# aosokin/os2d

Measured on AMD Instinct MI355X. Metric: query-image-pairs/s (1280-px input, ResNet50, N-class), higher is better.
Workload: dtype fftx3 (as fft; the per-bin complex GEMM on the fp16 MFMA with spectra split into fp16 hi+lo, 3 MFMAs per product, fp32 accumulate)

## Files before the change

include/os2d_hip.h:

```cpp
#ifndef OS2D_HIP_H
#define OS2D_HIP_H

#include <stddef.h>

#ifdef __cplusplus
extern "C" {
#endif

#define OS2D_ABI_VERSION 9

#define OS2D_PRECISION_F32 0
#define OS2D_PRECISION_F16X3 1
#define OS2D_PRECISION_F16X2 2

#define OS2D_PRECISION_FFT 3

#define OS2D_PRECISION_FFT32 5

#define OS2D_PRECISION_FFTX3 4

int os2d_abi_version(void);

const char* os2d_last_error(void);

// ... 20 lines not shown
int os2d_pack_conv_f16x3(int layer , int P, const float* w, const float* b, const float* bn_weight,
                         const float* bn_bias, const float* bn_running_mean, const float* bn_running_var, float bn_eps,
                         const int* weight_exp, const int* in_exp, const int* out_exp, void* packed_w, float* packed_b,
                         void* stream);

size_t os2d_class_split_bytes(int B, int C);
int os2d_class_split(const float* qp, void* qs, int B, int C, void* stream);

#define OS2D_STATUS_F16_RANGE 1
int os2d_head_forward_ex(const float* fm, const float* qp, const void* w1, const float* b1, const void* w2,
                         const float* b2, const void* w3, const float* b3, int A, int B, int C, int H, int W, int P,
                         int inverse, int stride, int rec_field, float* loc, float* cls, float* corners,
                         void* workspace, size_t workspace_bytes, void* stream, int precision, const void* qs,
                         void** stage_events, int* chunk_classes, int* status, const float* wspec, const float* twQ,
                         const float* twP);
void os2d_debug_set_dump(void* stream, int slot, void* dst, size_t bytes);
int os2d_prof_event_create(void** ev);
int os2d_prof_event_destroy(void* ev);
int os2d_prof_event_elapsed_ms(void* begin, void* end, float* ms);

int os2d_fm_sumsq(const float* fm, float* sumsq, int A, int C, int H, int W, void* stream);
size_t os2d_plane_floats(int H, int W);
int os2d_corr(const float* fm, const float* qp, const float* sumsq, float* corr, float* rnorm, int A, int B, int C,
              int H, int W, void* stream);
size_t os2d_corr_f16x3_workspace_bytes(int A, int C, int H, int W);
int os2d_corr_f16x3(const float* fm, const void* qs, float* corr, void* rshb, int A, int B, int C, int H, int W,
                    void* workspace, size_t workspace_bytes, void* stream);
size_t os2d_corr_f16x3_packed_workspace_bytes(int A, int B, int C, int H, int W);
int os2d_corr_f16x3_packed(const float* fm, const void* qs, float* corr, float* inv_norm, int A, int B, int C, int H, int W,
                           int form, void* workspace, size_t workspace_bytes, void* stream);
// ... 47 lines not shown
size_t os2d_spectral_weight16_bytes(int C, int nbins);
int os2d_spectral_weights_build(const double* wfold, const double* twP64, const double* twQ64, int C, int Cout, int P, int Q,
                                int nbins, int split, void* out, void* workspace, void* stream);
float os2d_spectral_xscale(int H, int W);
int os2d_spectral_gemm_f16(const void* w16, const float* X, float* Y, int NB, int C, int Cout, int nbins, float xscale,
                           void* stream);

int os2d_dft_sizes(int H, int W, int* P, int* Q, int* nbins, int* tiles);
int os2d_dft_channel_stride(int C);
size_t os2d_dft_matrices_bytes(int P, int Q);
int os2d_dft_matrices_build(const double* twP64, const double* twQ64, int P, int Q, void* out, void* stream);
int os2d_dft_forward(const float* corr, const float* inv_norm, float* X, const void* matrices, int NB, int C, int H, int W,
                     void* stream);
int os2d_dft_inverse(const float* Y, const float* packed_b, void* out, const void* matrices, int NB, int Cout, int H, int W,
                     int* status, void* stream);
int os2d_spectral_weights_build_dft(const double* wfold, const double* twP64, const double* twQ64, int C, int Cout, int P, int Q,
                                    int nbins, void* out, void* workspace, void* stream);
int os2d_spectral_gemm_f16_quads(const void* w16, const float* X, float* Y, int NB, int C, int Cout, int nbins, float xscale,
                                 void* stream);
float os2d_dft_xscale(int H, int W);

#define OS2D_PYRAMID_MAX_LEVELS 16
int os2d_detect_pyramid_supported(int L, int N, int nms_max_batch);
int os2d_detect_pyramid_workspace_bytes(int B, int N, int passes, size_t* bytes);
int os2d_detect_pyramid(const float* const* loc, const float* const* cls, const float* const* corners, int B, int L,
                        const int* hw, int stride, int rec_field, const float* img_wh, const float* scale_xy,
                        float score_threshold, float iou_threshold, int nms_max_batch, int passes, float* out_boxes,
                        float* out_scores, int* out_index, float* out_default, float* out_corners, int* out_count,
                        int* unfinished, void* workspace, size_t workspace_bytes, void* stream);
int os2d_detect_pyramid_merged(const float* const* loc, const float* const* cls, const float* const* corners, int B, int L,
// ... 19 lines not shown
```

os2d_amd/_lib.py:

```python
import ctypes

from . import build
from ._native import NativeLibrary, Os2dLibraryError

ABI_VERSION = 9

_c_float_p = ctypes.c_void_p
_vp = ctypes.c_void_p
_i = ctypes.c_int
_f = ctypes.c_float
_sz = ctypes.c_size_t

SIGNATURES = {
    "os2d_abi_version": (_i, []),
    "os2d_last_error": (ctypes.c_char_p, []),
    "os2d_packed_conv_floats": (_sz, [_i]),
    "os2d_packed_bias_floats": (_sz, [_i]),
    "os2d_pack_conv": (_i, [_i, _i, _vp, _vp, _vp, _vp, _vp, _vp, _f, _vp, _vp, _vp]),
    "os2d_class_prepare": (_i, [_vp, _i, _i, _i, _i, _vp, _vp, _vp]),
    "os2d_head_workspace_bytes": (_i, [_i, _i, _i, _i, _i, _i, ctypes.POINTER(_sz)]),
    "os2d_head_forward": (_i, [_vp] * 8 + [_i] * 9 + [_vp, _vp, _vp, _vp, _sz, _vp]),
    "os2d_packed_conv_bytes": (_sz, [_i, _i]),
    "os2d_pack_conv_f16x3": (_i, [_i, _i, _vp, _vp, _vp, _vp, _vp, _vp, _f, _vp, _vp, _vp, _vp, _vp, _vp]),
    "os2d_rnorm_exp": (_i, []),
# ... 16 lines not shown
    "os2d_fft_inverse": (_i, [_vp, _vp, _vp, _vp, _vp, _i, _i, _i, _i, _vp, _vp]),
    "os2d_fft_inverse_ex": (_i, [_vp, _vp, _vp, _vp, _vp, _i, _i, _i, _i, _vp, _i, _vp]),
    "os2d_dft_sizes": (_i, [_i, _i, ctypes.POINTER(_i), ctypes.POINTER(_i), ctypes.POINTER(_i), ctypes.POINTER(_i)]),
    "os2d_dft_channel_stride": (_i, [_i]),
    "os2d_dft_matrices_bytes": (_sz, [_i, _i]),
    "os2d_dft_matrices_build": (_i, [_vp, _vp, _i, _i, _vp, _vp]),
    "os2d_dft_forward": (_i, [_vp, _vp, _vp, _vp, _i, _i, _i, _i, _vp]),
    "os2d_dft_inverse": (_i, [_vp, _vp, _vp, _vp, _i, _i, _i, _i, _vp, _vp]),
    "os2d_spectral_weights_build_dft": (_i, [_vp, _vp, _vp, _i, _i, _i, _i, _i, _vp, _vp, _vp]),
    "os2d_spectral_gemm_f16_quads": (_i, [_vp, _vp, _vp, _i, _i, _i, _i, _f, _vp]),
    "os2d_dft_xscale": (_f, [_i, _i]),
    "os2d_class_split": (_i, [_vp, _vp, _i, _i, _vp]),
    "os2d_class_split_bytes": (_sz, [_i, _i]),
    "os2d_head_forward_ex": (_i, [_vp] * 8 + [_i] * 9 + [_vp, _vp, _vp, _vp, _sz, _vp, _i, _vp,
                                  ctypes.POINTER(_vp), ctypes.POINTER(_i), _vp, _vp, _vp, _vp]),
    "os2d_head_workspace_bytes_ex": (_i, [_i, _i, _i, _i, _i, _i, _i, ctypes.POINTER(_sz)]),
    "os2d_prof_event_create": (_i, [ctypes.POINTER(_vp)]),
    "os2d_prof_event_destroy": (_i, [_vp]),
    "os2d_prof_event_elapsed_ms": (_i, [_vp, _vp, ctypes.POINTER(_f)]),
    "os2d_fm_sumsq": (_i, [_vp, _vp, _i, _i, _i, _i, _vp]),
    "os2d_plane_floats": (_sz, [_i, _i]),
    "os2d_corr": (_i, [_vp, _vp, _vp, _vp, _vp, _i, _i, _i, _i, _i, _vp]),
    "os2d_corr_normalize": (_i, [_vp, _vp, _i, _i, _i, _vp]),
    "os2d_corr_f16x3_workspace_bytes": (_sz, [_i, _i, _i, _i]),
    "os2d_corr_f16x3": (_i, [_vp, _vp, _vp, _vp, _i, _i, _i, _i, _i, _vp, _sz, _vp]),
    "os2d_corr_f16x3_packed_workspace_bytes": (_sz, [_i, _i, _i, _i, _i]),
    "os2d_corr_f16x3_packed": (_i, [_vp, _vp, _vp, _vp, _i, _i, _i, _i, _i, _i, _vp, _sz, _vp]),
    "os2d_transform_conv": (_i, [_i, _vp, _vp, _vp, _vp, _i, _i, _i, _i, _vp]),
    "os2d_sample_decode": (_i, [_vp, _vp, _i, _i, _i, _i, _i, _i, _i, _vp, _vp, _vp, _vp]),
    "os2d_decode_boxes": (_i, [_vp, _i, _i, _i, _i, _i, _f, _f, _vp, _vp]),
# ... 43 lines not shown
```

os2d_amd/csrc/abi.hip:

```cpp
#include <stdio.h>

#include "../../include/os2d_hip.h"
#include "os2d_common.h"
#include "detect_common.h"
#include <atomic>
#include <mutex>
#include <random>
#include <vector>

namespace {
struct ConvShape {
  int cout, cin, ks, mt;
};
bool conv_shape(int layer, int P, ConvShape* s) {
  switch (layer) {
    case 1: *s = {128, OS2D_K, 7, 128}; return true;
    case 2: *s = {64, 128, 5, 64}; return true;
    case 3: *s = {P, 64, 5, 32}; return true;
    default: return false;
  }
}
size_t align_up(size_t x, size_t a) { return (x + a - 1) / a * a; }

int os2d_conv1_steps_padded() { return 25; }
// ... 366 lines not shown
  if (!boxes || !counts || !keep || !num_keep || !workspace || NC < 1 || N < 1) {
    os2d_set_error("os2d_nms: bad arguments");
    return -1;
  }
  if ((reinterpret_cast<uintptr_t>(boxes) & 15) || (reinterpret_cast<uintptr_t>(workspace) & 15)) {
    os2d_set_error("os2d_nms: boxes and workspace must be 16-byte aligned");
    return -1;
  }
  if (workspace_bytes < (size_t)NC * N * 4 * sizeof(float)) {
    os2d_set_error("os2d_nms: workspace too small");
    return -2;
  }
  return os2d_launch_nms(boxes, counts, NC, N, iou_threshold, keep, num_keep, workspace, os2d_stream(stream));
}

int os2d_head_forward_ex(const float* fm, const float* qp, const void* w1, const float* b1, const void* w2,
                         const float* b2, const void* w3, const float* b3, int A, int B, int C, int H, int W, int P,
                         int inverse, int stride, int rec_field, float* loc, float* cls, float* corners,
                         void* workspace, size_t workspace_bytes, void* stream, int precision, const void* qs,
                         void** stage_events, int* chunk_classes, int* status, const float* wspec, const float* twQ,
                         const float* twP) {
  if (!fm || !qp || !w1 || !b1 || !w2 || !b2 || !w3 || !b3 || !loc || !cls || !corners || !workspace) {
    os2d_set_error("os2d_head_forward: null pointer");
    return -1;
  }
  if (precision != OS2D_PRECISION_F32 && precision != OS2D_PRECISION_F16X3 && precision != OS2D_PRECISION_F16X2 &&
      precision != OS2D_PRECISION_FFT && precision != OS2D_PRECISION_FFTX3 && precision != OS2D_PRECISION_FFT32) {
    os2d_set_error("os2d_head_forward: unknown precision %d", precision);
    return -1;
  }
  int fft_bins = 0, tiles[6] = {1, 1, 0, 0, 0, 0};
  const bool dft = precision == OS2D_PRECISION_FFTX3;
  if (is_freq(precision)) {
    if (!wspec || !twQ || (!dft && !twP)) {
      os2d_set_error("os2d_head_forward: the frequency-domain modes need the weight spectra and the transform tables "
                     "(fft / fft32: twQ, twP; fftx3: the matrices of os2d_dft_matrices_build as twQ)");
      return -1;
    }
    if (!freq_plan(precision, H, W, nullptr, nullptr, &fft_bins, tiles)) {
      os2d_set_error("os2d_head_forward: no transform plan for a %dx%d map", H, W);
      return -3;
    }
  } else if (!direct7_width_ok(W)) {
    return -1;
  }
  const int fft_T = tiles[0] * tiles[1], xch = dft ? OS2D_XSPEC_CPAD : OS2D_K;
  const bool fp32_ops = precision == OS2D_PRECISION_F32 || precision == OS2D_PRECISION_FFT32;
  if (!fp32_ops && !qs) {
    os2d_set_error("os2d_head_forward: precision f16x3 / f16x2 needs the split class operand (os2d_class_split)");
    return -1;
  }
  if (!head_args_ok(A, B, C, H, W, P)) return -1;
  if (stride < 1 || rec_field < 1) {
    os2d_set_error("os2d_head_forward: bad stride/rec_field %d/%d", stride, rec_field);
    return -1;
  }
  if (reinterpret_cast<uintptr_t>(workspace) & 255) {
    os2d_set_error("os2d_head_forward: workspace must be 256-byte aligned");
    return -1;
  }
  const size_t one = carve(A, 1, C, H, W, P, fft_bins, fft_T, xch).total;
// ... 52 lines not shown
    } else {
      if ((rc = os2d_launch_corr(fm, qp + (size_t)b0 * C * OS2D_QROWS, sumsq, corr, fft_bins ? nullptr : rpad, invn, A, bc, C, H, W,
                                 0, st)))
        return rc;
    }
    mark(b0, 1);
    mark(b0, 2);
    if (fft_bins) {
      bool inv_borders = false;
      if (f16) {
        static const bool borders_in_inverse = [] {
          const char* e = getenv("OS2D_BORDERS_IN_INVERSE");
          return !(e && e[0] == '0');
        }();
        inv_borders = dft && borders_in_inverse;
        const int planes = inv_borders ? 0 : NB * 16 * 2;
        if ((planes || sumfx) &&
            (rc = os2d_launch_border_zero_shb_planes_norms(h1, planes, H, W, sumfx, invn, (size_t)NB * H * W, st)))
          return rc;
      } else if ((rc = os2d_launch_border_zero(h1, NB * 128, H, W, st))) {
        return rc;
      }
      mark(b0, 10);
      const int layout = precision == OS2D_PRECISION_FFTX3 ? OS2D_SPECTRA_QUADS : OS2D_SPECTRA_ROWS;
      if (dft) {
        const void* mats = twQ;
        if ((rc = os2d_launch_dft_forward(corr, invn, xspec, mats, NB, OS2D_K, xch, H, W, st))) return rc;
        mark(b0, 11);
        if ((rc = os2d_launch_spectral_gemm_f16(wspec, xspec, yspec, NB * fft_T, OS2D_K, 128, fft_bins,
                                                os2d_spectral_xscale_for(tiles[4], tiles[5]), 1, xch, st)))
          return rc;
        mark(b0, 12);
        if ((rc = os2d_launch_dft_inverse(yspec, b1, 128, h1, mats, NB, 128, H, W, whole_call, inv_borders ? 1 : 0, st))) return rc;
      } else {
        if ((rc = os2d_launch_fft_forward(corr, invn, xspec, twQ, twP, NB, OS2D_K, H, W, st))) return rc;
        mark(b0, 11);
        if ((rc = os2d_launch_spectral_gemm(wspec, xspec, yspec, NB * fft_T, OS2D_K, 128, fft_bins, st))) return rc;
        mark(b0, 12);
        if ((rc = os2d_launch_fft_inverse(yspec, b1, 128, h1, twQ, twP, NB, 128, H, W, whole_call, layout, f16 ? 0 : 1, st))) return rc;
      }
    } else if (f16) {
      if ((rc = os2d_launch_conv_f16x3(1, rpad, w1, b1, whole_call, h1, NB, P, H, W, terms1, st))) return rc;
    } else {
      if ((rc = os2d_launch_conv(1, rpad, static_cast<const float*>(w1), b1, h1, NB, P, H, W, st))) return rc;
    }
    mark(b0, 3);
    mark(b0, 4);
    if (dumps_active() && b0 == 0) {
      const size_t PLb = os2d_plane(H, W);
      dump_slot(stream, 0, corr, (size_t)NB * OS2D_K * H * W * 4);
      if (fft_bins) {
        dump_slot(stream, 1, invn, (size_t)NB * H * W * 4);
        dump_slot(stream, 2, xspec, (size_t)NB * fft_T * OS2D_K * fft_bins * 8);
        dump_slot(stream, 3, yspec, (size_t)NB * fft_T * 128 * fft_bins * 8);
      }
      dump_slot(stream, 4, h1, (size_t)NB * 128 * PLb * 4);
    }
    if (f16) {
      if ((rc = os2d_launch_conv_f16x3(2, h1, w2, b2, whole_call, h2, NB, P, H, W, 3, st))) return rc;
    } else {
      if ((rc = os2d_launch_conv(2, h1, static_cast<const float*>(w2), b2, h2, NB, P, H, W, st))) return rc;
    }
    mark(b0, 5);
    mark(b0, 6);
    if (dumps_active() && b0 == 0) dump_slot(stream, 5, h2, (size_t)NB * 64 * os2d_plane(H, W) * 4);
    static const bool fused_tail_env = [] {
      const char* e = getenv("OS2D_FUSED_TAIL");
      return !(e && e[0] == '0');
    }();
    const bool fused_tail = f16 && fused_tail_env && !dumps_active();
    if (fused_tail) {
      if ((rc = os2d_launch_conv3_sample_decode(h2, w3, b3, corr, NB, H, W, P, inverse, stride, rec_field, bc, B, b0, loc, cls, corners,
                                                flags, epoch, status, st)))
// ... 7 lines not shown
      if ((rc = os2d_launch_conv_f16x3(3, h2, w3, b3, whole_call, params, NB, P, H, W, 3, st))) return rc;
    } else {
      if ((rc = os2d_launch_conv(3, h2, static_cast<const float*>(w3), b3, params, NB, P, H, W, st))) return rc;
    }
    mark(b0, 7);
    mark(b0, 8);
    if (dumps_active() && b0 == 0) dump_slot(stream, 6, params, (size_t)NB * P * H * W * 4);
    if ((rc = os2d_launch_sample_decode(corr, params, NB, H, W, P, inverse, stride, rec_field, bc, B, b0, loc, cls,
                                        corners, fp32_ops ? nullptr : flags, epoch, status, st)))
      return rc;
    mark(b0, 9);
  }
  return 0;
}

int os2d_head_forward(const float* fm, const float* qp, const float* w1, const float* b1, const float* w2,
                      const float* b2, const float* w3, const float* b3, int A, int B, int C, int H, int W, int P,
                      int inverse, int stride, int rec_field, float* loc, float* cls, float* corners, void* workspace,
                      size_t workspace_bytes, void* stream) {
  return os2d_head_forward_ex(fm, qp, w1, b1, w2, b2, w3, b3, A, B, C, H, W, P, inverse, stride, rec_field, loc, cls,
                              corners, workspace, workspace_bytes, stream, OS2D_PRECISION_F32, nullptr, nullptr, nullptr,
                              nullptr, nullptr, nullptr, nullptr);
}

size_t os2d_class_split_bytes(int B, int C) {
  if (B < 1 || C < 1) return 0;
  return (size_t)B * os2d_corr_groups(C) * 2 * 256 * 16;
}

int os2d_class_split(const float* qp, void* qs, int B, int C, void* stream) {
// ... 186 lines not shown
size_t os2d_dft_matrices_bytes(int P, int Q) {
  if (P < 4 || (P & 3) || Q < 2 || (Q & 1)) return 0;
  return os2d_dft_matrices_size(P, Q);
}

int os2d_dft_matrices_build(const double* twP64, const double* twQ64, int P, int Q, void* out, void* stream) {
  if (!twP64 || !twQ64 || !out || (reinterpret_cast<uintptr_t>(out) & 15)) {
    os2d_set_error("os2d_dft_matrices_build: bad arguments (out must be 16-byte aligned)");
    return -1;
  }
  return os2d_launch_dft_matrices(twP64, twQ64, P, Q, out, os2d_stream(stream));
}

int os2d_dft_forward(const float* corr, const float* inv_norm, float* X, const void* matrices, int NB, int C, int H, int W,
                     void* stream) {
  if (!corr || !inv_norm || !X || !matrices || NB < 1 || C < 1 || H < 1 || W < 1) {
    os2d_set_error("os2d_dft_forward: bad arguments");
    return -1;
  }
  return os2d_launch_dft_forward(corr, inv_norm, X, matrices, NB, C, os2d_dft_channel_stride(C), H, W, os2d_stream(stream));
}

int os2d_dft_inverse(const float* Y, const float* packed_b, void* out, const void* matrices, int NB, int Cout, int H, int W,
                     int* status, void* stream) {
  if (!Y || !packed_b || !out || !matrices || NB < 1 || Cout != 128 || H < 1 || W < 1) {
    os2d_set_error("os2d_dft_inverse: bad arguments (Cout must be 128: the 7x7 layer)");
    return -1;
  }
  return os2d_launch_dft_inverse(Y, packed_b, 128, out, matrices, NB, Cout, H, W, Os2dRangeFlag{status, OS2D_STATUS_F16_RANGE}, 1, os2d_stream(stream));
}

int os2d_spectral_weights_build_dft(const double* wfold, const double* twP64, const double* twQ64, int C, int Cout, int P, int Q,
                                    int nbins, void* out, void* workspace, void* stream) {
  if (!wfold || !twP64 || !twQ64 || !out || !workspace || C < 1 || Cout < 1 || Cout > 128 || nbins < 8 || (nbins & 7) || (P & 3)) {
    os2d_set_error("os2d_spectral_weights_build_dft: bad arguments (C=%d Cout=%d P=%d nbins=%d)", C, Cout, P, nbins);
    return -1;
  }
  if ((reinterpret_cast<uintptr_t>(out) & 15) || (reinterpret_cast<uintptr_t>(workspace) & 7)) {
    os2d_set_error("os2d_spectral_weights_build_dft: out must be 16-byte, workspace 8-byte aligned");
    return -1;
  }
  return os2d_launch_spectra_pack(wfold, twP64, twQ64, C, Cout, P, Q, nbins, 1, 1, out, workspace, os2d_stream(stream));
}

// ... 50 lines not shown
```

os2d_amd/csrc/dft_mfma.h:

```cpp
#pragma once

#ifndef DFT_DEV
#error "the includer defines DFT_DEV, DFT_TID, DFT_BID, DFT_GRID, DFT_LDS, DFT_BARRIER, DFT_MFMA, DFT_SHFL_XOR, DFT_SHFL_XOR_U32, DFT_BALLOT, DFT_FLAG, DFT_FLAG_SET, DFT_RAISE, DFT_UNIFORM"
#endif

#ifndef DFT_HD
#define DFT_HD static inline
#endif
#ifndef DFT_MEMBER
#define DFT_MEMBER inline
#endif
#ifndef DFT_LANDED
#define DFT_LANDED(X)
#endif
#ifndef DFT_FWD_PREFETCH_AFTER
#define DFT_FWD_PREFETCH_AFTER 2
#endif
#ifndef DFT_INV_PREFETCH_AFTER
#define DFT_INV_PREFETCH_AFTER 2
#endif
#ifndef DFT_PIPE_REGA
#define DFT_PIPE_REGA 1
#endif
#ifndef DFT_PIPE_LDS
// ... 11 lines not shown
#define DFT_STAMP_END(BASE)
#endif

#include "tile_common.h"

namespace os2d_dft {

typedef float f32x4u __attribute__((ext_vector_type(4), aligned(4)));

constexpr int DFT_THR = 512, DFT_WAVES = 8;
constexpr int DFT_G = 4;
constexpr int DFT_MAXP = 64;
constexpr int DFT_MAXV = 48;
constexpr int DFT_MAXWK = 96;
constexpr int DFT_KREG = 8;

struct DftPlan {
  int H, W;
  int P, Q, V, NBINS;
  int T, TY, TX, TH, TW;
  int oy, ox;
  int LH, LW;
  int RH;
  int Pp;
  int Wk;
  int N1;
  int M2;
  int Mx;
  int N2;
  int MA;
// ... 357 lines not shown

template <bool TILED, bool FAST, int G, int NW, int KS2 = 0>
DFT_DEV void dft_forward_body(const float* corr,
                              const float* invn,
                              float* X,
                              const u32x4* FqT, const u32x4* Fp2, const DftPlan& pl, int C, int Cpad, int NBT, int iters) {
  constexpr int THR = NW * 64;
  constexpr bool ALDS = G == 8;
  constexpr bool R2 = !ALDS && KS2 == 8;
  unsigned char* smem = DFT_LDS;
  const int tid = DFT_TID, lane = tid & 63, l31 = lane & 31, hw = lane >> 5;
  const int wv = DFT_UNIFORM(tid >> 6);
  const int P = pl.P, V = pl.V, Pp = pl.Pp, Wk = pl.Wk, N1 = pl.N1, Mx = pl.Mx, N2 = pl.N2, LH = pl.LH, LW = pl.LW, W = pl.W, H = pl.H;
  const int MxS = Mx + 1, N2S = N2 + 1;
  const int CG = (C + G - 1) / G, HW = H * W;
  u32x4* ldsF = reinterpret_cast<u32x4*>(smem);
  u32x4* ldsU = reinterpret_cast<u32x4*>(smem + pl.lds_const);
  unsigned char* ldsUb = smem + pl.lds_const;
  const int nF = (Wk / 8) * 2 * N1;
  for (int i = tid; i < nF; i += THR) ldsF[i] = FqT[i];
  const unsigned char* ldsTw = smem + pl.lds_const + pl.lds_union + DFT_R2_LDS_TW;
  if (R2 && tid < DFT_R2_TWU) reinterpret_cast<u32x4*>(smem + pl.lds_const + pl.lds_union + DFT_R2_LDS_TW)[tid] = Fp2[DFT_R2_MATU + tid];
  u32x4* ldsP = ldsF + nF;
  if (ALDS)
    for (int i = tid; i < (2 * Pp / 8) * 2 * pl.M2; i += THR) ldsP[i] = Fp2[i];

  const int mt1n = Mx / 32, nt1n = N1 / 32, nt2n = N2 / 32, mt2n = pl.M2 / 32;
  const int ks1n = Wk / 16, ks2n = 2 * Pp / 16;
  const int mt2 = wv & 3;
  constexpr int KR2 = R2 ? 4 : KS2 ? KS2 : DFT_KREG;
// ... 25 lines not shown
  f32x4 pc[NSLOT][G], pn[NSLOT];
#define DFT_FWD_ITER(IT)                                                                                     \
  const int pr_ = dft_div((IT), pl.inv_cg), cg_ = (IT)-pr_ * CG;                                             \
  const int nb_ = TILED ? dft_div(pr_, pl.inv_t) : pr_, tile_ = TILED ? pr_ - nb_ * pl.T : 0;               \
  const int ty_ = TILED ? dft_div(tile_, pl.inv_tx) : 0, tx_ = TILED ? tile_ - ty_ * pl.TX : 0;             \
  const int Y0 = TILED ? ty_ * pl.TH - pl.oy : 0, X0 = TILED ? tx_ * pl.TW - pl.ox : 0;                     \
  const int c0_ = cg_ * G;
#define DFT_FWD_POS(TID, S)                                                                                  \
  const int i_ = (TID) + (S)*THR;                                                                        \
  const int r_ = dft_div(i_, pl.inv_c4), c4_ = i_ - r_ * (Wk / 4);                                          \
  const int y_ = Y0 + r_, x_ = X0 + 4 * c4_;
#define DFT_FWD_PREFETCH(IT, TID) DFT_FWD_PREFETCH_SLOTS(IT, TID, 0, NSLOT)
#define DFT_FWD_PREFETCH_SLOTS(IT, TID, S0, S1)                                                              \
  {                                                                                                          \
    DFT_FWD_ITER(IT)                                                                                         \
    _Pragma("unroll") for (int s = (S0); s < (S1); ++s) {                                                    \
      DFT_FWD_POS(TID, s)                                                                                    \
      if (FAST) {                                                                                            \
        const bool ok = i_ < npos && r_ < LH && 4 * c4_ < LW;                                                \
        const int off = ok ? y_ * W + x_ : 0;                                                                \
        pn[s] = *reinterpret_cast<const f32x4*>(invn + (size_t)nb_ * HW + off);                             \
        _Pragma("unroll") for (int g = 0; g < G; ++g) {                                                  \
          const int c = c0_ + g < C ? c0_ + g : C - 1;                                                       \
          pc[s][g] = *reinterpret_cast<const f32x4*>(corr + ((size_t)nb_ * C + c) * HW + off);              \
        }                                                                                                    \
      } else {                                                                                               \
                                                                           \
        const bool rok = i_ < npos && r_ < LH && y_ >= 0 && y_ < H;                                          \
        const int off0 = y_ * W + x_;                                                                        \
        const bool vec = rok && off0 >= 0 && off0 + 3 < HW;                                                  \
        const int offv = vec ? off0 : 0;                                                                     \
        pn[s] = *reinterpret_cast<const f32x4u*>(invn + (size_t)nb_ * HW + offv);                            \
        _Pragma("unroll") for (int g = 0; g < G; ++g) {                                                      \
          const int c = c0_ + g < C ? c0_ + g : C - 1;                                                       \
          pc[s][g] = *reinterpret_cast<const f32x4u*>(corr + ((size_t)nb_ * C + c) * HW + offv);             \
        }                                                                                                    \
        if (rok && !vec) {                                                                                   \
          _Pragma("unroll") for (int e = 0; e < 4; ++e) {                                                    \
            const bool ok = 4 * c4_ + e < LW && x_ + e >= 0 && x_ + e < W;                                   \
            const int off = ok ? y_ * W + x_ + e : 0;                                                        \
            pn[s][e] = invn[(size_t)nb_ * HW + off];                                                         \
            _Pragma("unroll") for (int g = 0; g < G; ++g) {                                                  \
              const int c = c0_ + g < C ? c0_ + g : C - 1;                                                   \
              pc[s][g][e] = corr[((size_t)nb_ * C + c) * HW + off];                                          \
            }                                                                                                \
          }                                                                                                  \
        }                                                                                                    \
      }                                                                                                      \
    }                                                                                                        \
  }
  const int first = (DFT_GRID & 7) == 0 ? (DFT_BID & 7) * (DFT_GRID >> 3) + (DFT_BID >> 3) : DFT_BID;
  if (first < iters) DFT_FWD_PREFETCH(first, tid)
  DFT_BARRIER();

  DFT_STAMP_BEGIN()
  for (int it = first; it < iters; it += DFT_GRID) {
    int tl = tid;
#ifndef OS2D_HOST_EMU
    asm volatile("" : "+v"(tl));
#endif
    const int lane = tl & 63, l31 = lane & 31, hw = lane >> 5;
    DFT_FWD_ITER(it)
    {
#pragma unroll
      for (int s = 0; s < NSLOT; ++s) {
        DFT_FWD_POS(tl, s)
        if (i_ < npos) {
          float nsc[4];
#pragma unroll
          for (int e = 0; e < 4; ++e) {
            const bool ok = FAST ? (r_ < LH && 4 * c4_ < LW) : (r_ < LH && y_ >= 0 && y_ < H && 4 * c4_ + e < LW && x_ + e >= 0 && x_ + e < W);
            nsc[e] = ok ? pn[s][e] * 32768.0f : 0.f;
          }
#pragma unroll
          for (int g = 0; g < G; ++g) {
            u32x2 hi = {0u, 0u}, lo = {0u, 0u};
            if (c0_ + g < C)
              dft_split4(fmaxf(pc[s][g][0], 0.f) * nsc[0], fmaxf(pc[s][g][1], 0.f) * nsc[1], fmaxf(pc[s][g][2], 0.f) * nsc[2],
                         fmaxf(pc[s][g][3], 0.f) * nsc[3], &hi, &lo);
            const int m = g * Pp + (R2 ? (r_ & 1) * 32 + (r_ >> 1) : r_);
            unsigned char* dst = ldsUb + ((size_t)((c4_ >> 1) * 2) * MxS + m) * 16 + (c4_ & 1) * 8;
            *reinterpret_cast<u32x2*>(dst) = hi;
            *reinterpret_cast<u32x2*>(dst + (size_t)MxS * 16) = lo;
          }
        }
      }
      for (int i = tid; i < (Mx - G * Pp) * (Wk / 8) * 2; i += THR) {
// ... 379 lines not shown
#pragma unroll
    for (int j = 0; j < 3; ++j) {
      const int t = wv + DFT_WAVES * j;
      const bool mine = t < mtBn * ntBn;
      bn[j] = mine ? t / mtBn : 0;
      bm[j] = mine ? t - bn[j] * mtBn : -1;
      ntbw += mine ? 1 : 0;
#pragma unroll
      for (int r = 0; r < 16; ++r) yc[j][r] = 0.f;
    }
    dft_product_lds_any<DFT_WAVES, DFT_PIPE_LDS ? 1 : 0>(yc, ntbw, 0, ksBn, ldsU, MBS, ldsG, NBo, wv, mtBn, l31, hw);
    DFT_INV_MAXIMA(tl)
    DFT_STAMP(4)

    {
      float bias[4], osc[4];
#pragma unroll
      for (int g = 0; g < 4; ++g) {
        bias[g] = bp[o0 + (G == 8 ? 4 * hw : 0) + g];
        osc[g] = bp[2 * MTP + o0 + (G == 8 ? 4 * hw : 0) + g];
      }
      const int grp = o0 >> 3, slot = o0 & 7;
      unsigned char* hi_unit = out + (((size_t)nb * ((Cout + 7) >> 3) + grp) * 2 + 0) * (size_t)PLANE * 16 + slot * 2;
      unsigned char* lo_unit = out + (((size_t)nb * ((Cout + 7) >> 3) + grp) * 2 + 1) * (size_t)PLANE * 16 + slot * 2;
      if (zero_borders && (!TILED || tile == 0)) {
        const int rows = H * (Ws - W), tail0 = BASE + H * Ws, npad = BASE + rows + (PLANE - tail0);
        for (int k = tl; k < npad; k += DFT_THR) {
          int cell;
          if (k < BASE) cell = k;
          else if (k < BASE + rows) {
            const int jj = k - BASE, hr = jj / (Ws - W);
            cell = BASE + hr * Ws + W + (jj - hr * (Ws - W));
          } else cell = tail0 + (k - BASE - rows);
          if (G == 8) {
            *reinterpret_cast<u32x4*>(hi_unit + (size_t)cell * 16) = u32x4{0u, 0u, 0u, 0u};
            *reinterpret_cast<u32x4*>(lo_unit + (size_t)cell * 16) = u32x4{0u, 0u, 0u, 0u};
          } else {
            *reinterpret_cast<u32x2*>(hi_unit + (size_t)cell * 16) = u32x2{0u, 0u};
            *reinterpret_cast<u32x2*>(lo_unit + (size_t)cell * 16) = u32x2{0u, 0u};
          }
// ... 3 lines not shown
      for (int j = 0; j < 3; ++j) {
        if (bm[j] < 0) continue;
        const int wwin = bn[j] * 32 + l31, tw = wwin - ox;
#pragma unroll
        for (int q = 0; q < 4; ++q) {
          const int hwin = G == 8 ? bm[j] * 4 + q : (bm[j] * 32 + 8 * q + 4 * hw) >> 2, th = hwin - oy;
          const int h = y0 + th, w = x0 + tw;
          const bool inside = th >= 0 && th < TH_ && tw >= 0 && tw < TW_ && h < H && w < W;
          if (G == 8 || inside) {
            float t[4];
#pragma unroll
            for (int g = 0; g < 4; ++g) {
              const float pre = yc[j][4 * q + g] * cinv[g] + bias[g];
              t[g] = fmaxf(pre, 0.f) * osc[g];
              if (inside && (!(fabsf(t[g]) <= 65504.f) || pre != pre)) bad = true;
            }
            u32x2 hi, lo;
            dft_split4(t[0], t[1], t[2], t[3], &hi, &lo);
            const size_t off = ((size_t)BASE + (size_t)h * Ws + w) * 16;
            if (G == 8) {
              const u32x2 send = hw ? hi : lo, keep = hw ? lo : hi;
              u32x2 recv;
              recv[0] = DFT_SHFL_XOR_U32(send[0], 32);
              recv[1] = DFT_SHFL_XOR_U32(send[1], 32);
              const u32x4 unit = hw ? u32x4{recv[0], recv[1], keep[0], keep[1]} : u32x4{keep[0], keep[1], recv[0], recv[1]};
              if (inside) *reinterpret_cast<u32x4*>((hw ? lo_unit : hi_unit) + off) = unit;
            } else {
              *reinterpret_cast<u32x2*>(hi_unit + off) = hi;
              *reinterpret_cast<u32x2*>(lo_unit + off) = lo;
            }
// ... 19 lines not shown
```

os2d_amd/csrc/os2d_common.h:

```cpp
#pragma once
#include <hip/hip_runtime.h>
#include <stdint.h>

#include "../csrc_shared/abi_common.h"

#define OS2D_PAD 3
#define OS2D_T 15
#define OS2D_K 225
#define OS2D_KP 226
#define OS2D_QROWS 256
#define OS2D_MAX_W_DIRECT7 209
#define OS2D_MAX_W_LINEAR5 316
#define OS2D_MAX_W 3600
#define OS2D_MAX_H 2784
#define OS2D_XSPEC_CPAD 232
#define OS2D_G 29
#define OS2D_RNORM_EXP 12
#define OS2D_STATUS_F16_RANGE 1

struct Os2dRangeFlag {
  int* word;
  int value;
};
#ifdef __HIPCC__
// ... 86 lines not shown
                             int NBINS, int split, int u_fastest ,
                             void* out, void* workspace, hipStream_t stream);
size_t os2d_spectral_weight_floats(int C, int Cout, int NBINS);
int os2d_launch_spectral_gemm(const float* wspec, const float* X, float* Y, int NB, int C, int Cout, int NBINS,
                              hipStream_t stream);
size_t os2d_spectral_weight16_size(int C, int NBINS);
float os2d_spectral_xscale_for(int H, int W);
int os2d_launch_spectral_gemm_f16(const void* w16, const float* X, float* Y, int NB, int C, int Cout, int NBINS, float xscale,
                                  int x_quads , int Cpad,
                                  hipStream_t stream);
int os2d_dft_plan(int H, int W, int* P, int* Q, int* nbins, int* tiles );
size_t os2d_dft_matrices_size(int P, int Q);
int os2d_launch_dft_matrices(const double* twP64, const double* twQ64, int P, int Q, void* out, hipStream_t stream);
int os2d_launch_dft_forward(const float* corr, const float* inv, float* X, const void* matrices, int NB, int C, int Cpad, int H, int W,
                            hipStream_t stream);
int os2d_launch_dft_inverse(const float* Y, const float* bp, int MTP, void* out, const void* matrices, int NB, int Cout, int H, int W,
                            Os2dRangeFlag status, int zero_borders, hipStream_t stream);
int os2d_corr_groups(int C);
int os2d_launch_split_fm(const float* fm, const float* sumsq, void* fs, int A, int C, int HW, void* clear, size_t clear_words,
                         Os2dRangeFlag status, hipStream_t stream);
int os2d_launch_split_qp(const float* qp, void* qs, int B, int C, hipStream_t stream);
int os2d_launch_corr_f16x3(const void* fs, const void* qs, float* corr, void* rshb, float* invn, void* sumfx, int flags, int A,
                           int B, int C, int H, int W, hipStream_t stream);
int os2d_corr_f16x3_use_packed(int A, int B, int H, int W);
int os2d_launch_corr_sums_clear(void* sumfx, int A, int B, int H, int W, hipStream_t stream);
```

os2d_amd/modeling/head.py:

```python
import collections
import itertools
import ctypes
import logging
import os

import torch
import torch.nn as nn

from .. import _lib
from ..structures.feature_map import FeatureMapSize
from .box_coder import BoxGridGenerator
from . import head_train

TEMPLATE = 15
QROWS = 256
MAX_W_DIRECT7 = 209
FFT_MIN_PAIRS = 7
PRECISIONS = {"f32": 0, "f16x3": 1, "f16x2": 2, "fft": 3, "fftx3": 4, "fft32": 5}
FFT_MODES = ("fft", "fftx3", "fft32")
FP32_MODES = ("f32", "fft32")
DEFAULT_PRECISION = "fftx3"


def resolve_precision(precision=None):
# ... 312 lines not shown
        def out_exp(bound):
            return floor_log2(32768.0 / bound.clamp_min(1e-300)) * (bound > 0).to(torch.int32)

        def weight_exp(w, in_exp):
            eff = w * torch.exp2(-in_exp.double()).view(1, -1, 1, 1)
            amax = eff.abs().amax(dim=(1, 2, 3))
            return floor_log2(16384.0 / amax.clamp_min(1e-300)) * (amax > 0).to(torch.int32)

        lib = _lib.load()
        bound1 = 7.0 * w1.flatten(1).norm(dim=1) + b1.abs()
        l1 = (w2.abs().sum(dim=(2, 3)) * bound1.view(1, -1)).sum(dim=1)
        l2 = 5.0 * bound1.norm() * w2.flatten(1).norm(dim=1)
        bound2 = torch.minimum(l1, l2) + b2.abs()
        e0 = torch.full((225,), lib.os2d_rnorm_exp(), dtype=torch.int32, device=w1.device)
        e1, e2 = out_exp(bound1), out_exp(bound2)
        return dict(in_exp=[e0, e1, e2], out_exp=[e1, e2, None],
                    weight_exp=[weight_exp(w1, e0), weight_exp(w2, e1), weight_exp(w3, e2)], bounds=(bound1, bound2))

    def packed(self, precision=None):
        precision = resolve_precision(precision)
        if precision in ("f16x2", "fft", "fftx3"):
            precision = "f16x3"
        elif precision == "fft32":
            precision = "f32"
        key = (precision,) + self._state_key()
        dev = self.linear.weight.device
        cached = self._packed_cache.get(precision)
        if cached is not None and cached.key == key:
            return cached.get(dev)
        lib = _lib.load()
        self.check_ready()
# ... 75 lines not shown
                wspec = torch.empty(lib.os2d_spectral_weight_bytes(225, 128, nbins) // 4, dtype=torch.float32, device=dev)
                _lib.check(lib.os2d_spectral_weights_build(_lib.ptr(wfold), _lib.ptr(tp64), _lib.ptr(tq64), 225, 128, P, Q, nbins,
                                                           0, _lib.ptr(wspec), _lib.ptr(scratch), stream), "os2d_spectral_weights_build")

                def table(n):
                    m = torch.arange(n, dtype=torch.float64)
                    ang = -2.0 * torch.pi * m / n
                    return torch.stack([torch.cos(ang), torch.sin(ang)], 1).float().to(dev).contiguous()
                result = (wspec, table(Q), table(P), nbins)
            cur = torch.cuda.current_stream(dev)
            for t in (wfold, tp64, tq64, scratch):
                t.record_stream(cur)
            store.put(self._net_id, slot, _StreamOrdered(key, result, dev))
        return result

    @property
    def _spectra_cache(self):
        dev = self.linear.weight.device
        if dev.type != "cuda":
            return {}
        store = _SpectraStore.of(dev)
        return _SpectraView(store, self._net_id)

    def forward(self, corr_maps, precision="f32"):
        corr_maps = _require_device_f32(corr_maps, "corr_maps")
        if corr_maps.dim() != 4 or corr_maps.size(1) != 225:
            raise RuntimeError("corr_maps must be [N,225,H,W], got {}".format(tuple(corr_maps.shape)))
        if torch.is_grad_enabled() and (corr_maps.requires_grad or any(p.requires_grad for p in self.parameters())) and self.training:
            raise RuntimeError("autograd through the HIP TransformNet is not implemented (training is out of scope)")
        precision = resolve_precision(precision)
# ... 252 lines not shown
        lib = _lib.load()
        dev = feature_maps.device
        regressor = self.aligner.parameter_regressor
        P = regressor.output_dim
        precision, pinned = _resolve(precision or self.precision)
        regressor.check_ready()
        spectra = None
        if W > MAX_W_DIRECT7:
            precision = {"f32": "fft32", "f16x3": "fftx3", "f16x2": "fftx3"}.get(precision, precision)
            pinned = True
        if precision in FFT_MODES:
            pairs = A * B if route_pairs is None else int(route_pairs)
            spectra = regressor.spectra(H, W, split=precision == "fftx3") if (pinned or pairs >= FFT_MIN_PAIRS) else None
            if spectra is None:
                precision = "f32" if precision == "fft32" else "f16x3"
        self.last_precision = precision
        w1, b1, w2, b2, w3, b3 = regressor.packed(precision)
        if out is None:
            loc = torch.empty(A, B, 4, H, W, dtype=torch.float32, device=dev)
            cls = torch.empty(A, B, 1, H, W, dtype=torch.float32, device=dev)
            corners = torch.empty(A, B, 8, H, W, dtype=torch.float32, device=dev)
        else:
            loc, cls, corners = out
            for t, k in ((loc, 4), (cls, 1), (corners, 8)):
                if tuple(t.shape) != (A, B, k, H, W) or not t.is_contiguous() or t.device != dev or t.dtype != torch.float32:
                    raise RuntimeError("out tensors must be contiguous float32 [A,B,{},H,W] on {}".format(k, dev))
        full = ctypes.c_size_t()
        one = ctypes.c_size_t()
        _lib.check(lib.os2d_head_workspace_bytes_ex(A, B, C, H, W, P, PRECISIONS[precision], ctypes.byref(full)), "os2d_head_workspace_bytes_ex")
        _lib.check(lib.os2d_head_workspace_bytes_ex(A, 1, C, H, W, P, PRECISIONS[precision], ctypes.byref(one)), "os2d_head_workspace_bytes_ex")
        with torch.cuda.device(dev):
            ws = get_workspace(dev, full.value, one.value)
            status = self._status_word() if precision not in FP32_MODES else None
            _lib.check(lib.os2d_head_forward_ex(
                _lib.ptr(feature_maps), _lib.ptr(self._qp), _lib.ptr(w1), _lib.ptr(b1), _lib.ptr(w2), _lib.ptr(b2),
                _lib.ptr(w3), _lib.ptr(b3), A, B, C, H, W, P, 1 if self.aligner.use_inverse_geom_model else 0,
                self._stride, self._rec_field, _lib.ptr(loc), _lib.ptr(cls), _lib.ptr(corners),
                _lib.ptr(ws), ws.numel(), _lib.current_stream(dev), PRECISIONS[precision],
                _lib.ptr(self._split_class_operand()) if precision not in FP32_MODES else None, stage_events, None,
                _lib.host_ptr(status), *([_lib.ptr(t) for t in spectra[:3]] if spectra is not None else [None, None, None])),
                "os2d_head_forward_ex")
        strict = self.strict_range if strict_range is None else strict_range
        if strict and precision not in FP32_MODES:
            torch.cuda.current_stream(dev).synchronize()
            if int(self._status[0]) != 0:
                self.clear_range_status()
                logging.getLogger("OS2D").warning("OS2D head: non-finite input or an activation outside the fp16 range; strict_range "
                                                  "re-runs this call in precision='f32'")
                return self.forward(feature_maps, out=out, stage_events=stage_events, precision="f32")
        return loc, cls, cls, corners


def normalize_feature_map_L2(feature_maps, epsilon=1e-6):
    return feature_maps / (feature_maps.norm(dim=1, keepdim=True) + epsilon)
```

Baseline: 45120.

## Compute the 5x5 conv2 layer in the frequency domain via DFT and spectral GEMM

Adds a frequency-domain path for the second head convolution (128->64, 5x5). The first layer's inverse DFT now writes plain fp32 planes, which are forward-DFT'd with unit norm, multiplied by precomputed conv2 weight spectra, and inverse-transformed into the split hi/lo layout with borders. The aim is to replace the direct f16x3 conv2 with cheaper per-bin complex GEMMs. The cost is extra transforms, an fp32 intermediate buffer, and a cached weight spectrum per size. It is on by default for fftx3 and can be turned off with an environment variable.

```diff
diff --git a/include/os2d_hip.h b/include/os2d_hip.h
--- a/include/os2d_hip.h
+++ b/include/os2d_hip.h
@@ -58,6 +58,12 @@
                          void* workspace, size_t workspace_bytes, void* stream, int precision, const void* qs,
                          void** stage_events, int* chunk_classes, int* status, const float* wspec, const float* twQ,
                          const float* twP);
+int os2d_head_forward_ex2(const float* fm, const float* qp, const void* w1, const float* b1, const void* w2,
+                          const float* b2, const void* w3, const float* b3, int A, int B, int C, int H, int W, int P,
+                          int inverse, int stride, int rec_field, float* loc, float* cls, float* corners,
+                          void* workspace, size_t workspace_bytes, void* stream, int precision, const void* qs,
+                          void** stage_events, int* chunk_classes, int* status, const float* wspec, const float* twQ,
+                          const float* twP, const void* wspec2);
 void os2d_debug_set_dump(void* stream, int slot, void* dst, size_t bytes);
 int os2d_prof_event_create(void** ev);
 int os2d_prof_event_destroy(void* ev);
@@ -135,6 +141,8 @@
                      void* stream);
 int os2d_dft_inverse(const float* Y, const float* packed_b, void* out, const void* matrices, int NB, int Cout, int H, int W,
                      int* status, void* stream);
+int os2d_dft_inverse_planes(const float* Y, const float* packed_b, float* out, const void* matrices, int NB, int Cout, int H, int W,
+                            int* status, void* stream);
 int os2d_spectral_weights_build_dft(const double* wfold, const double* twP64, const double* twQ64, int C, int Cout, int P, int Q,
                                     int nbins, void* out, void* workspace, void* stream);
 int os2d_spectral_gemm_f16_quads(const void* w16, const float* X, float* Y, int NB, int C, int Cout, int nbins, float xscale,
diff --git a/os2d_amd/_lib.py b/os2d_amd/_lib.py
--- a/os2d_amd/_lib.py
+++ b/os2d_amd/_lib.py
@@ -54,6 +54,9 @@
     "os2d_class_split_bytes": (_sz, [_i, _i]),
     "os2d_head_forward_ex": (_i, [_vp] * 8 + [_i] * 9 + [_vp, _vp, _vp, _vp, _sz, _vp, _i, _vp,
                                   ctypes.POINTER(_vp), ctypes.POINTER(_i), _vp, _vp, _vp, _vp]),
+    "os2d_head_forward_ex2": (_i, [_vp] * 8 + [_i] * 9 + [_vp, _vp, _vp, _vp, _sz, _vp, _i, _vp,
+                                   ctypes.POINTER(_vp), ctypes.POINTER(_i), _vp, _vp, _vp, _vp, _vp]),
+    "os2d_dft_inverse_planes": (_i, [_vp, _vp, _vp, _vp, _i, _i, _i, _i, _vp, _vp]),
     "os2d_head_workspace_bytes_ex": (_i, [_i, _i, _i, _i, _i, _i, _i, ctypes.POINTER(_sz)]),
     "os2d_prof_event_create": (_i, [ctypes.POINTER(_vp)]),
     "os2d_prof_event_destroy": (_i, [_vp]),
diff --git a/os2d_amd/csrc/abi.hip b/os2d_amd/csrc/abi.hip
--- a/os2d_amd/csrc/abi.hip
+++ b/os2d_amd/csrc/abi.hip
@@ -404,12 +404,12 @@
   return os2d_launch_nms(boxes, counts, NC, N, iou_threshold, keep, num_keep, workspace, os2d_stream(stream));
 }
 
-int os2d_head_forward_ex(const float* fm, const float* qp, const void* w1, const float* b1, const void* w2,
-                         const float* b2, const void* w3, const float* b3, int A, int B, int C, int H, int W, int P,
-                         int inverse, int stride, int rec_field, float* loc, float* cls, float* corners,
-                         void* workspace, size_t workspace_bytes, void* stream, int precision, const void* qs,
-                         void** stage_events, int* chunk_classes, int* status, const float* wspec, const float* twQ,
-                         const float* twP) {
+int os2d_head_forward_ex2(const float* fm, const float* qp, const void* w1, const float* b1, const void* w2,
+                          const float* b2, const void* w3, const float* b3, int A, int B, int C, int H, int W, int P,
+                          int inverse, int stride, int rec_field, float* loc, float* cls, float* corners,
+                          void* workspace, size_t workspace_bytes, void* stream, int precision, const void* qs,
+                          void** stage_events, int* chunk_classes, int* status, const float* wspec, const float* twQ,
+                          const float* twP, const void* wspec2) {
   if (!fm || !qp || !w1 || !b1 || !w2 || !b2 || !w3 || !b3 || !loc || !cls || !corners || !workspace) {
     os2d_set_error("os2d_head_forward: null pointer");
     return -1;
@@ -435,6 +435,11 @@
     return -1;
   }
   const int fft_T = tiles[0] * tiles[1], xch = dft ? OS2D_XSPEC_CPAD : OS2D_K;
+  static const bool conv2_freq_env = [] {
+    const char* e = getenv("OS2D_CONV2_FREQ");
+    return !(e && e[0] == '0');
+  }();
+  const bool conv2_freq = dft && wspec2 && conv2_freq_env;
   const bool fp32_ops = precision == OS2D_PRECISION_F32 || precision == OS2D_PRECISION_FFT32;
   if (!fp32_ops && !qs) {
     os2d_set_error("os2d_head_forward: precision f16x3 / f16x2 needs the split class operand (os2d_class_split)");
@@ -517,7 +522,7 @@
           return !(e && e[0] == '0');
         }();
         inv_borders = dft && borders_in_inverse;
-        const int planes = inv_borders ? 0 : NB * 16 * 2;
+        const int planes = (inv_borders || conv2_freq) ? 0 : NB * 16 * 2;
         if ((planes || sumfx) &&
             (rc = os2d_launch_border_zero_shb_planes_norms(h1, planes, H, W, sumfx, invn, (size_t)NB * H * W, st)))
           return rc;
@@ -534,7 +539,9 @@
                                                 os2d_spectral_xscale_for(tiles[4], tiles[5]), 1, xch, st)))
           return rc;
         mark(b0, 12);
-        if ((rc = os2d_launch_dft_inverse(yspec, b1, 128, h1, mats, NB, 128, H, W, whole_call, inv_borders ? 1 : 0, st))) return rc;
+        if ((rc = os2d_launch_dft_inverse(yspec, b1, 128, h1, mats, NB, 128, H, W, whole_call,
+                                          conv2_freq ? OS2D_DFT_OUT_PLANES : inv_borders ? OS2D_DFT_OUT_SHB_BORDERS : OS2D_DFT_OUT_SHB, st)))
+          return rc;
       } else {
         if ((rc = os2d_launch_fft_forward(corr, invn, xspec, twQ, twP, NB, OS2D_K, H, W, st))) return rc;
         mark(b0, 11);
@@ -557,9 +564,15 @@
         dump_slot(stream, 2, xspec, (size_t)NB * fft_T * OS2D_K * fft_bins * 8);
         dump_slot(stream, 3, yspec, (size_t)NB * fft_T * 128 * fft_bins * 8);
       }
-      dump_slot(stream, 4, h1, (size_t)NB * 128 * PLb * 4);
+      dump_slot(stream, 4, h1, (size_t)NB * 128 * (conv2_freq ? (size_t)H * W : PLb) * 4);
     }
-    if (f16) {
+    if (conv2_freq) {
+      if ((rc = os2d_launch_dft_forward(h1, nullptr, xspec, twQ, NB, 128, 128, H, W, st))) return rc;
+      if ((rc = os2d_launch_spectral_gemm_f16(wspec2, xspec, yspec, NB * fft_T, 128, 64, fft_bins,
+                                              os2d_spectral_xscale_for(tiles[4], tiles[5]), 1, 128, st)))
+        return rc;
+      if ((rc = os2d_launch_dft_inverse(yspec, b2, 64, h2, twQ, NB, 64, H, W, whole_call, OS2D_DFT_OUT_SHB_BORDERS, st))) return rc;
+    } else if (f16) {
       if ((rc = os2d_launch_conv_f16x3(2, h1, w2, b2, whole_call, h2, NB, P, H, W, 3, st))) return rc;
     } else {
       if ((rc = os2d_launch_conv(2, h1, static_cast<const float*>(w2), b2, h2, NB, P, H, W, st))) return rc;
@@ -597,6 +610,16 @@
   return 0;
 }
 
+int os2d_head_forward_ex(const float* fm, const float* qp, const void* w1, const float* b1, const void* w2,
+                         const float* b2, const void* w3, const float* b3, int A, int B, int C, int H, int W, int P,
+                         int inverse, int stride, int rec_field, float* loc, float* cls, float* corners,
+                         void* workspace, size_t workspace_bytes, void* stream, int precision, const void* qs,
+                         void** stage_events, int* chunk_classes, int* status, const float* wspec, const float* twQ,
+                         const float* twP) {
+  return os2d_head_forward_ex2(fm, qp, w1, b1, w2, b2, w3, b3, A, B, C, H, W, P, inverse, stride, rec_field, loc, cls, corners, workspace,
+                               workspace_bytes, stream, precision, qs, stage_events, chunk_classes, status, wspec, twQ, twP, nullptr);
+}
+
 int os2d_head_forward(const float* fm, const float* qp, const float* w1, const float* b1, const float* w2,
                       const float* b2, const float* w3, const float* b3, int A, int B, int C, int H, int W, int P,
                       int inverse, int stride, int rec_field, float* loc, float* cls, float* corners, void* workspace,
@@ -813,7 +836,7 @@
 
 int os2d_dft_forward(const float* corr, const float* inv_norm, float* X, const void* matrices, int NB, int C, int H, int W,
                      void* stream) {
-  if (!corr || !inv_norm || !X || !matrices || NB < 1 || C < 1 || H < 1 || W < 1) {
+  if (!corr || !X || !matrices || NB < 1 || C < 1 || H < 1 || W < 1) {
     os2d_set_error("os2d_dft_forward: bad arguments");
     return -1;
   }
@@ -822,11 +845,22 @@
 
 int os2d_dft_inverse(const float* Y, const float* packed_b, void* out, const void* matrices, int NB, int Cout, int H, int W,
                      int* status, void* stream) {
-  if (!Y || !packed_b || !out || !matrices || NB < 1 || Cout != 128 || H < 1 || W < 1) {
-    os2d_set_error("os2d_dft_inverse: bad arguments (Cout must be 128: the 7x7 layer)");
-    return -1;
-  }
-  return os2d_launch_dft_inverse(Y, packed_b, 128, out, matrices, NB, Cout, H, W, Os2dRangeFlag{status, OS2D_STATUS_F16_RANGE}, 1, os2d_stream(stream));
+  if (!Y || !packed_b || !out || !matrices || NB < 1 || (Cout != 128 && Cout != 64) || H < 1 || W < 1) {
+    os2d_set_error("os2d_dft_inverse: bad arguments (Cout must be 128 or 64: the 7x7 layer / the 5x5 layer 128 -> 64)");
+    return -1;
+  }
+  return os2d_launch_dft_inverse(Y, packed_b, Cout, out, matrices, NB, Cout, H, W, Os2dRangeFlag{status, OS2D_STATUS_F16_RANGE},
+                                 OS2D_DFT_OUT_SHB_BORDERS, os2d_stream(stream));
+}
+
+int os2d_dft_inverse_planes(const float* Y, const float* packed_b, float* out, const void* matrices, int NB, int Cout, int H, int W,
+                            int* status, void* stream) {
+  if (!Y || !packed_b || !out || !matrices || NB < 1 || (Cout != 128 && Cout != 64) || H < 1 || W < 1) {
+    os2d_set_error("os2d_dft_inverse_planes: bad arguments (Cout must be 128 or 64)");
+    return -1;
+  }
+  return os2d_launch_dft_inverse(Y, packed_b, Cout, out, matrices, NB, Cout, H, W, Os2dRangeFlag{status, OS2D_STATUS_F16_RANGE},
+                                 OS2D_DFT_OUT_PLANES, os2d_stream(stream));
 }
 
 int os2d_spectral_weights_build_dft(const double* wfold, const double* twP64, const double* twQ64, int C, int Cout, int P, int Q,
diff --git a/os2d_amd/csrc/dft_mfma.h b/os2d_amd/csrc/dft_mfma.h
--- a/os2d_amd/csrc/dft_mfma.h
+++ b/os2d_amd/csrc/dft_mfma.h
@@ -49,6 +49,7 @@
 constexpr int DFT_MAXV = 48;
 constexpr int DFT_MAXWK = 96;
 constexpr int DFT_KREG = 8;
+constexpr int DFT_OUT_SHB = 0, DFT_OUT_SHB_BORDERS = 1, DFT_OUT_PLANES = 2;
 
 struct DftPlan {
   int H, W;
@@ -436,6 +437,7 @@
   const int P = pl.P, V = pl.V, Pp = pl.Pp, Wk = pl.Wk, N1 = pl.N1, Mx = pl.Mx, N2 = pl.N2, LH = pl.LH, LW = pl.LW, W = pl.W, H = pl.H;
   const int MxS = Mx + 1, N2S = N2 + 1;
   const int CG = (C + G - 1) / G, HW = H * W;
+  const bool unit_norm = invn == nullptr;
   u32x4* ldsF = reinterpret_cast<u32x4*>(smem);
   u32x4* ldsU = reinterpret_cast<u32x4*>(smem + pl.lds_const);
   unsigned char* ldsUb = smem + pl.lds_const;
@@ -491,12 +493,14 @@
 #define DFT_FWD_PREFETCH_SLOTS(IT, TID, S0, S1)                                                              \
   {                                                                                                          \
     DFT_FWD_ITER(IT)                                                                                         \
+     \
+    const float* nrm_ = invn ? invn + (size_t)nb_ * HW : corr + ((size_t)nb_ * C + (c0_ < C ? c0_ : C - 1)) * HW; \
     _Pragma("unroll") for (int s = (S0); s < (S1); ++s) {                                                    \
       DFT_FWD_POS(TID, s)                                                                                    \
       if (FAST) {                                                                                            \
         const bool ok = i_ < npos && r_ < LH && 4 * c4_ < LW;                                                \
         const int off = ok ? y_ * W + x_ : 0;                                                                \
-        pn[s] = *reinterpret_cast<const f32x4*>(invn + (size_t)nb_ * HW + off);                             \
+        pn[s] = *reinterpret_cast<const f32x4*>(nrm_ + off);                                                \
         _Pragma("unroll") for (int g = 0; g < G; ++g) {                                                  \
           const int c = c0_ + g < C ? c0_ + g : C - 1;                                                       \
           pc[s][g] = *reinterpret_cast<const f32x4*>(corr + ((size_t)nb_ * C + c) * HW + off);              \
@@ -507,7 +511,7 @@
         const int off0 = y_ * W + x_;                                                                        \
         const bool vec = rok && off0 >= 0 && off0 + 3 < HW;                                                  \
         const int offv = vec ? off0 : 0;                                                                     \
-        pn[s] = *reinterpret_cast<const f32x4u*>(invn + (size_t)nb_ * HW + offv);                            \
+        pn[s] = *reinterpret_cast<const f32x4u*>(nrm_ + offv);                                               \
         _Pragma("unroll") for (int g = 0; g < G; ++g) {                                                      \
           const int c = c0_ + g < C ? c0_ + g : C - 1;                                                       \
           pc[s][g] = *reinterpret_cast<const f32x4u*>(corr + ((size_t)nb_ * C + c) * HW + offv);             \
@@ -516,7 +520,7 @@
           _Pragma("unroll") for (int e = 0; e < 4; ++e) {                                                    \
             const bool ok = 4 * c4_ + e < LW && x_ + e >= 0 && x_ + e < W;                                   \
             const int off = ok ? y_ * W + x_ + e : 0;                                                        \
-            pn[s][e] = invn[(size_t)nb_ * HW + off];                                                         \
+            pn[s][e] = nrm_[off];                                                                            \
             _Pragma("unroll") for (int g = 0; g < G; ++g) {                                                  \
               const int c = c0_ + g < C ? c0_ + g : C - 1;                                                   \
               pc[s][g][e] = corr[((size_t)nb_ * C + c) * HW + off];                                          \
@@ -547,7 +551,7 @@
 #pragma unroll
           for (int e = 0; e < 4; ++e) {
             const bool ok = FAST ? (r_ < LH && 4 * c4_ < LW) : (r_ < LH && y_ >= 0 && y_ < H && 4 * c4_ + e < LW && x_ + e >= 0 && x_ + e < W);
-            nsc[e] = ok ? pn[s][e] * 32768.0f : 0.f;
+            nsc[e] = ok ? (unit_norm ? 32768.0f : pn[s][e] * 32768.0f) : 0.f;
           }
 #pragma unroll
           for (int g = 0; g < G; ++g) {
@@ -957,6 +961,7 @@
     DFT_STAMP(4)
 
     {
+      const bool planes = zero_borders == DFT_OUT_PLANES;
       float bias[4], osc[4];
 #pragma unroll
       for (int g = 0; g < 4; ++g) {
@@ -966,7 +971,7 @@
       const int grp = o0 >> 3, slot = o0 & 7;
       unsigned char* hi_unit = out + (((size_t)nb * ((Cout + 7) >> 3) + grp) * 2 + 0) * (size_t)PLANE * 16 + slot * 2;
       unsigned char* lo_unit = out + (((size_t)nb * ((Cout + 7) >> 3) + grp) * 2 + 1) * (size_t)PLANE * 16 + slot * 2;
-      if (zero_borders && (!TILED || tile == 0)) {
+      if (zero_borders == DFT_OUT_SHB_BORDERS && (!TILED || tile == 0)) {
         const int rows = H * (Ws - W), tail0 = BASE + H * Ws, npad = BASE + rows + (PLANE - tail0);
         for (int k = tl; k < npad; k += DFT_THR) {
           int cell;
@@ -1000,6 +1005,14 @@
               const float pre = yc[j][4 * q + g] * cinv[g] + bias[g];
               t[g] = fmaxf(pre, 0.f) * osc[g];
               if (inside && (!(fabsf(t[g]) <= 65504.f) || pre != pre)) bad = true;
+            }
+            if (planes) {
+              if (inside) {
+                float* dst = reinterpret_cast<float*>(out) + ((size_t)nb * Cout + o0 + (G == 8 ? 4 * hw : 0)) * ((size_t)H * W) + (size_t)h * W + w;
+#pragma unroll
+                for (int g = 0; g < 4; ++g) dst[(size_t)g * H * W] = t[g] * (1.0f / 32768.0f);
+              }
+              continue;
             }
             u32x2 hi, lo;
             dft_split4(t[0], t[1], t[2], t[3], &hi, &lo);
diff --git a/os2d_amd/csrc/os2d_common.h b/os2d_amd/csrc/os2d_common.h
--- a/os2d_amd/csrc/os2d_common.h
+++ b/os2d_amd/csrc/os2d_common.h
@@ -124,8 +124,9 @@
 int os2d_launch_dft_matrices(const double* twP64, const double* twQ64, int P, int Q, void* out, hipStream_t stream);
 int os2d_launch_dft_forward(const float* corr, const float* inv, float* X, const void* matrices, int NB, int C, int Cpad, int H, int W,
                             hipStream_t stream);
+enum { OS2D_DFT_OUT_SHB = 0, OS2D_DFT_OUT_SHB_BORDERS = 1, OS2D_DFT_OUT_PLANES = 2 };
 int os2d_launch_dft_inverse(const float* Y, const float* bp, int MTP, void* out, const void* matrices, int NB, int Cout, int H, int W,
-                            Os2dRangeFlag status, int zero_borders, hipStream_t stream);
+                            Os2dRangeFlag status, int form, hipStream_t stream);
 int os2d_corr_groups(int C);
 int os2d_launch_split_fm(const float* fm, const float* sumsq, void* fs, int A, int C, int HW, void* clear, size_t clear_words,
                          Os2dRangeFlag status, hipStream_t stream);
diff --git a/os2d_amd/modeling/head.py b/os2d_amd/modeling/head.py
--- a/os2d_amd/modeling/head.py
+++ b/os2d_amd/modeling/head.py
@@ -350,7 +350,7 @@
         bound2 = torch.minimum(l1, l2) + b2.abs()
         e0 = torch.full((225,), lib.os2d_rnorm_exp(), dtype=torch.int32, device=w1.device)
         e1, e2 = out_exp(bound1), out_exp(bound2)
-        return dict(in_exp=[e0, e1, e2], out_exp=[e1, e2, None],
+        return dict(in_exp=[e0, e1, e2], out_exp=[e1, e2, None], unit_exp=e1 - 15,
                     weight_exp=[weight_exp(w1, e0), weight_exp(w2, e1), weight_exp(w3, e2)], bounds=(bound1, bound2))
 
     def packed(self, precision=None):
@@ -456,6 +456,43 @@
             store.put(self._net_id, slot, _StreamOrdered(key, result, dev))
         return result
 
+    def spectra2(self, H, W):
+        lib = _lib.load()
+        self.check_ready()
+        cP, cQ, cN = ctypes.c_int(), ctypes.c_int(), ctypes.c_int()
+        if lib.os2d_dft_sizes(int(H), int(W), ctypes.byref(cP), ctypes.byref(cQ), ctypes.byref(cN), None) != 0:
+            return None
+        P, Q, nbins = cP.value, cQ.value, cN.value
+        dev = self.linear.weight.device
+        key = self._state_key()
+        slot = (P, Q, True, "conv2")
+        store = _SpectraStore.of(dev)
+        cached = store.get(self._net_id, slot, key)
+        if cached is not None:
+            return cached.get(dev)
+        with torch.cuda.device(dev), torch.no_grad():
+            _, (w2, _), _ = self._folded()
+            unit_exp = self.range_plan()["unit_exp"].to(w2.device).double()
+            w2 = nn.functional.pad(w2 * torch.exp2(-unit_exp).view(1, -1, 1, 1), (1, 1, 1, 1))
+
+            def table64(n):
+                m = torch.arange(n, dtype=torch.float64)
+                ang = m * (-2.0 * torch.pi / n)
+                return torch.stack([torch.cos(ang), torch.sin(ang)], 1).to(dev).contiguous()
+            wfold = w2.to(dev).contiguous()
+            tp64, tq64 = table64(P), table64(Q)
+            scratch = torch.empty(1024, dtype=torch.uint8, device=dev)
+            stream = _lib.current_stream(dev)
+            wspec = torch.empty(lib.os2d_spectral_weight16_bytes(128, nbins), dtype=torch.uint8, device=dev)
+            _lib.check(lib.os2d_spectral_weights_build_dft(_lib.ptr(wfold), _lib.ptr(tp64), _lib.ptr(tq64), 128, 64, P, Q, nbins,
+                                                           _lib.ptr(wspec), _lib.ptr(scratch), stream),
+                       "os2d_spectral_weights_build_dft")
+            cur = torch.cuda.current_stream(dev)
+            for t in (wfold, tp64, tq64, scratch):
+                t.record_stream(cur)
+            store.put(self._net_id, slot, _StreamOrdered(key, wspec, dev))
+        return wspec
+
     @property
     def _spectra_cache(self):
         dev = self.linear.weight.device
@@ -738,6 +775,9 @@
             spectra = regressor.spectra(H, W, split=precision == "fftx3") if (pinned or pairs >= FFT_MIN_PAIRS) else None
             if spectra is None:
                 precision = "f32" if precision == "fft32" else "f16x3"
+        spectra2 = None
+        if precision == "fftx3" and spectra is not None and not os.environ.get("OS2D_CONV2_FREQ", "1").startswith("0"):
+            spectra2 = regressor.spectra2(H, W)
         self.last_precision = precision
         w1, b1, w2, b2, w3, b3 = regressor.packed(precision)
         if out is None:
@@ -756,14 +796,15 @@
         with torch.cuda.device(dev):
             ws = get_workspace(dev, full.value, one.value)
             status = self._status_word() if precision not in FP32_MODES else None
-            _lib.check(lib.os2d_head_forward_ex(
+            _lib.check(lib.os2d_head_forward_ex2(
                 _lib.ptr(feature_maps), _lib.ptr(self._qp), _lib.ptr(w1), _lib.ptr(b1), _lib.ptr(w2), _lib.ptr(b2),
                 _lib.ptr(w3), _lib.ptr(b3), A, B, C, H, W, P, 1 if self.aligner.use_inverse_geom_model else 0,
                 self._stride, self._rec_field, _lib.ptr(loc), _lib.ptr(cls), _lib.ptr(corners),
                 _lib.ptr(ws), ws.numel(), _lib.current_stream(dev), PRECISIONS[precision],
                 _lib.ptr(self._split_class_operand()) if precision not in FP32_MODES else None, stage_events, None,
-                _lib.host_ptr(status), *([_lib.ptr(t) for t in spectra[:3]] if spectra is not None else [None, None, None])),
-                "os2d_head_forward_ex")
+                _lib.host_ptr(status), *([_lib.ptr(t) for t in spectra[:3]] if spectra is not None else [None, None, None]),
+                _lib.ptr(spectra2)),
+                "os2d_head_forward_ex2")
         strict = self.strict_range if strict_range is None else strict_range
         if strict and precision not in FP32_MODES:
             torch.cuda.current_stream(dev).synchronize()
```

Result: faster. 45980, median of 6 (+1.9%).
